# nekopanda/Amatsukaze

Hardware: AMD Instinct MI355X
Metric: frames/sec 1440x1080i logo+CM+KFM pass (higher is better)
Workload: dtype f32; 1 GPU; configs[1]: 10000x 1440x1080i 8-bit in HBM: AMTAnalyzeLogo, LogoFrame scan x3, CM/KFM metrics, CalcFade, AMTEraseLogo; analysis_mode=linear, library_default_mode=exact, calc_fade=device, erase=into a resident writable copy (MakeWritable's frame), frames_per_gpu=10000, logo=256x128@(1120,64), parallelism=single GPU

## Files before the change

### amatsukaze_amd/build.py

```python
from __future__ import annotations

import os
import subprocess
import sys

HERE = os.path.dirname(os.path.abspath(__file__))
CSRC = os.path.join(HERE, "csrc")
OUT = os.path.join(HERE, "libamt_gpu.so")

SOURCES = [
    "amt_gpu.hip",
    "amt_gpu_erase_scan.hip",
    "amt_gpu_stats.hip",
    "amt_gpu_ingest.hip",
    "amt_gpu_upload.hip",
    "eval_engine.hip",
    "eval_fused_kernels.hip",
    "eval_linear_kernels.hip",
    "eval_pair_kernels.hip",
    "eval_pair1_kernels.hip",
    "erase_scan_kernels.hip",
    "erase_surface_kernels.hip",
    "stats_kernels.hip",
    "stats_msb_kernels.hip",
    "ingest_kernels.hip",
    "amt_gpu_logofind.hip",
    "logofind_kernels.hip",
    "logofind_msb_kernels.hip",
    "surface_kernels.hip",
    "amt_gpu_audio.hip",
    "audio_kernels.hip",
    "amt_gpu_render.hip",
    "render_kernels.hip",
    "render_surface_kernels.hip",
    "render_adaptive_kernels.hip",
    "render_adaptive_surface_kernels.hip",
    "amt_gpu_tnr.hip",
    "temporal_nr_kernels.hip",
    "temporal_nr_surface_kernels.hip",
    "amt_gpu_resize.hip",
    "resize_kernels.hip",
    "resize_surface_kernels.hip",
    "resize_plan.cpp",
    "amt_gpu_deband.hip",
    "deband_kernels.hip",
    "deband_surface_kernels.hip",
    "deband_plan.cpp",
    "amt_gpu_edgelevel.hip",
    "edgelevel_kernels.hip",
    "logo_model.cpp",
    "logo_fit.cpp",
    "decisions.cpp",
    "stats_decisions.cpp",
    "amts_file.cpp",
    "logo_find.cpp",
]

FLAGS = ["--offload-arch=gfx950", "-O3", "-std=c++17", "-fPIC", "-ffp-contract=off", "-fno-fast-math",
         "-fgpu-rdc" if False else "-fno-gpu-rdc", "-Wall", "-Wno-unused-function", "-Wno-unused-result"]


EXTRA_FLAGS = {"eval_fused_kernels.hip": ["-mllvm", "-amdgpu-sched-strategy=max-ilp"],
               "eval_linear_kernels.hip": ["-fno-slp-vectorize"]}


def hipcc() -> str:
    for c in (os.environ.get("HIPCC"), "/opt/rocm/bin/hipcc", "hipcc"):
        if c and (os.path.isabs(c) and os.path.exists(c) or not os.path.isabs(c)):
            return c
    raise RuntimeError("hipcc not found")


def needs_build(srcs) -> bool:
# ... 64 lines not shown
```

### amatsukaze_amd/csrc/engine.hpp

```cpp
#pragma once

#include <hip/hip_runtime.h>

#include <cstdint>
#include <mutex>
#include <utility>
#include <stdexcept>
#include <string>
#include <vector>

#include "eval_plan.h"
#include "eval_tiles.hpp"
#include "kernels.hpp"
#include "logo_model.hpp"

#define AMT_HIP(expr)                                                                              \
    do {                                                                                           \
        hipError_t e_ = (expr);                                                                    \
        if (e_ != hipSuccess)                                                                      \
            throw std::runtime_error(std::string(#expr) + ": " + hipGetErrorString(e_));          \
    } while (0)

#ifdef AMT_TRACE_CALLS
#include <chrono>
// ... 97 lines not shown
};

struct EvalLogoSpec {
    LogoPlanes planes;
    MaskTables tables;
    int imgx = 0, imgy = 0;
    int row0 = 0, row_step = 1, deint = 1;
    int out_off = 0;
};

class EvalEngine {
public:
    EvalEngine(AmtGpuContext* ctx, std::vector<EvalLogoSpec> specs, std::vector<float> fades, bool take_abs, int out_frame_stride,
               const char* prof_name = "logo_eval_fused_kernel");
    void run(const FrameBatch& luma, int bits, int nframes, float* dout, const int* dframe_map = nullptr);
    void run_linear(const FrameBatch& luma, int bits, int nframes, float* dout, const int* dframe_map = nullptr, uint8_t* dforce = nullptr);
    void set_linear_queue(int entries) { lin_queue_ = entries; }
    float linear_error_bound(int logo, int bits) const;
    void run_listed(const FrameBatch& luma, int bits, int max_frames, const int* dlist, const int* dcount, float* dout, int G = 1,
                    int fade_chunk = -1);
    int exact_group_frames(int nframes) const;
    int num_fades() const { return (int)fades_.size(); }
    int num_logos() const { return (int)specs_.size(); }
    const EvalLogoSpec& spec(int i) const { return specs_[i]; }
    double mask_pixel_evals_per_frame() const;

private:
    AmtGpuContext* ctx_;
    std::vector<EvalLogoSpec> specs_;
    std::vector<float> fades_;
    bool take_abs_;
    int out_frame_stride_;
    std::string prof_name_;
    int plane_cap_ = 0;
    int group_frames_ = 0;
    std::vector<EvalBand> bands_;
    std::vector<DevBuf<float>> d_a_, d_b_;
    std::vector<DevBuf<float2>> d_scales_, d_kslot_;
    std::vector<DevBuf<uint2>> d_slot2_;
    DevBuf<EvalLogoDev> d_logos_;
    DevBuf<EvalBand> d_bands_;
    DevBuf<float> d_fades_;
    bool pair_eligible();
    bool pair_addressable(int pitch_bytes) const;
    bool tiles_usable(int pitch_bytes) const;
    int pair_state_ = -1;
    void ensure_tiles();
    bool tiles_ready_ = false;
    bool tile_slots_ok_ = true;
    static bool stage4_eligible(const EvalLogoSpec& S);
    bool tiles_stage4_ = false;
    std::vector<DevBuf<float2>> d_tkp_, d_tsc_, d_tpq_;
    bool tiles_units_ = false;
    std::vector<DevBuf<uint32_t>> d_tinfo_, d_tpos_, d_tunits_;
    std::vector<DevBuf<char>> d_tlin_;
    int lin_queue_ = 256;
    std::vector<DevBuf<TileDesc>> d_tiles_;
    std::vector<DevBuf<TileBandDesc>> d_tbands_;
    std::vector<DevBuf<int>> d_tlist_;
    DevBuf<TileLogoDev> d_tls_;
    void ensure_linear();
    bool linear_ready_ = false;
    float vmax_unit_ = 1.0f;
    std::vector<double> lin_err_corr_, lin_err_sum_;
    std::vector<double> lin_err_formula_;
    bool lin_formula_ok_ = true;
};

}
```

### amatsukaze_amd/csrc/eval_engine.hip

```cpp
#include "build_knobs.h"
#include "engine.hpp"
#include "exact_math.h"

#include <algorithm>
#include <cmath>
#include <cstring>

int AmtGpuContext::prof_id(const char* name)
{
    for (size_t i = 0; i < prof_names.size(); ++i) if (prof_names[i] == name) return (int)i;
    prof_names.push_back(name);
    prof_ms.push_back(0.0);
    prof_calls.push_back(0);
    return (int)prof_names.size() - 1;
}
hipEvent_t AmtGpuContext::prof_event()
{
    if (!prof_pool.empty()) { hipEvent_t e = prof_pool.back(); prof_pool.pop_back(); return e; }
    hipEvent_t e;
    AMT_HIP(hipEventCreate(&e));
    return e;
}
int AmtGpuContext::prof_begin(const char* name)
{
// ... 110 lines not shown
            for (int sidx = B.s0; sidx < B.s0 + B.nslots; ++sidx) {
                const int m0 = slot_m0(sidx);
                const int n = (int)(slots[sidx] >> 28);
                const int x = (int)(T.pos[m0] & 0xFFFF), y = (int)(T.pos[m0] >> 16);
                slot2[sidx] = uint2{slots[sidx], (uint32_t)((y - 2 - B.y0) * B.lp + (x - 2 - B.x0))};
                const float* k0 = &T.kernels[(size_t)m0 * 25];
                const float* k1 = n > 1 ? &T.kernels[(size_t)(m0 + 1) * 25] : nullptr;
                for (int c = 0; c < 5; ++c)
                    for (int r = 0; r < 5; ++r) {
                        const float a0 = c < 4 ? k0[r * 5 + c + 1] : k0[r * 5];
                        const float a1 = k1 ? (c < 4 ? k1[r * 5 + c] : k1[r * 5 + 4]) : 0.0f;
                        kslot[(size_t)(c * 5 + r) * spad + sidx] = float2{a0, a1};
                    }
            }
        }
        d_a_[i].upload(S.planes.A(0), (size_t)w * h, ctx_->stream);
        d_b_[i].upload(S.planes.B(0), (size_t)w * h, ctx_->stream);
        d_scales_[i].upload(scales, ctx_->stream);
        d_kslot_[i].upload(kslot, ctx_->stream);
        d_slot2_[i].upload(slot2, ctx_->stream);

        EvalLogoDev& D = hl[i];
        D.a = d_a_[i].get(); D.b = d_b_[i].get(); D.scales = d_scales_[i].get();
        D.kslot = d_kslot_[i].get(); D.slot2 = d_slot2_[i].get(); D.nslots_pad = spad;
        D.band0 = band0; D.nbands = (int)bands_.size() - band0;
        D.w = w; D.h = h; D.count = T.count; D.count_pad = cpad;
        D.imgx = S.imgx; D.imgy = S.imgy; D.row0 = S.row0; D.row_step = S.row_step; D.deint = S.deint;
        D.blackScore = T.blackScore;
        D.out_off = S.out_off;
        D.lp = lp;
    }
    d_logos_.upload(hl, ctx_->stream);
    d_bands_.upload(bands_, ctx_->stream);
    d_fades_.upload(fades_, ctx_->stream);
}

double EvalEngine::mask_pixel_evals_per_frame() const
{
    double s = 0;
    for (const auto& sp : specs_) s += (double)sp.tables.count * fades_.size();
    return s;
}

void EvalEngine::run(const FrameBatch& luma, int bits, int nframes, float* dout, const int* dframe_map)
{
    if (nframes <= 0 || specs_.empty()) return;
    ctx_->bind();
    const int nl = (int)specs_.size();
    int G = exact_group_frames(nframes);
    const int nf_all = (int)fades_.size();
    if (pair_eligible() && pair_addressable(luma.pitchY * luma.es)) {
        const size_t dot = prof_name_.find('.');
        const std::string suffix = dot == std::string::npos ? std::string() : prof_name_.substr(dot);
        const int Gp = group_frames_ > 0 ? group_frames_ : (int)std::max(1LL, std::min((long long)kTileMaxFrames, (long long)nframes * nl / 2048));
        const int sp = ctx_->prof_begin(((tiles_stage4_ ? "logo_eval_pair_kernel" : "logo_eval_pair_ldexp_kernel") + suffix).c_str());
        AMT_HIP((tiles_units_ ? launch_logo_eval_pair1 : launch_logo_eval_pair)(ctx_->stream, bits, d_logos_.get(), d_tls_.get(), nl, luma, dframe_map, nframes, Gp, dout, out_frame_stride_,
                                      take_abs_ ? 1 : 0, tiles_stage4_ ? 0 : 1));
        ctx_->prof_end(sp);
        return;
    }
    for (int f0 = 0; f0 < nf_all; f0 += kEvalMaxFades) {
        const int nf = std::min(kEvalMaxFades, nf_all - f0);
        G = std::max(1, std::min(G, kEvalThreads / nf));
        const int sp = ctx_->prof_begin(prof_name_.c_str());
        AMT_HIP(launch_logo_eval_fused(ctx_->stream, bits, d_logos_.get(), nl, d_bands_.get(), d_fades_.get(), nf, f0, luma, dframe_map, nframes, G,
                                       dout, out_frame_stride_, take_abs_ ? 1 : 0, plane_cap_));
        ctx_->prof_end(sp);
    }
}

int EvalEngine::exact_group_frames(int nframes) const
{
    const int nl = (int)specs_.size();
    return group_frames_ > 0 ? group_frames_ : (int)std::max(1LL, std::min(8LL, (long long)nframes * nl / 2048));
}

bool EvalEngine::pair_eligible()
{
    if (pair_state_ >= 0) return pair_state_ == 1;
    pair_state_ = 0;
    if (fades_.size() != 2 || fades_[0] != 0.0f || fades_[1] != 1.0f || specs_.empty()) return false;
    for (const EvalLogoSpec& S : specs_) {
        const int w = S.planes.w, h = S.planes.h;
        if (w < 6 || (w & 1) || h < 5 || S.tables.count <= 0 || S.tables.count >= (1 << 20)) return false;
        if (!S.deint) return false;
        const float* a = S.planes.A(0);
        const float* b = S.planes.B(0);
        for (int p = 0; p < w * h; ++p)
            if (!(std::fabs(a[p]) + std::fabs(b[p]) < 8192.0f)) return false;
    }
    ensure_tiles();
    if (!tile_slots_ok_) return false;
    pair_state_ = 1;
    return true;
}

bool EvalEngine::pair_addressable(int pitch_bytes) const
{
    for (const EvalLogoSpec& S : specs_) {
        const long long last_row = (long long)S.imgy + S.row0 + (long long)S.planes.h * S.row_step + 1;
        const long long last = last_row * pitch_bytes + (long long)(S.imgx + S.planes.w) * 2;
        if (last >= (1LL << 31) || pitch_bytes <= 0) return false;
        if ((long long)S.imgy + S.row0 < 0 || !tile_mul24_operands_ok(pitch_bytes, S.row_step, last_row, S.planes.w, S.planes.h)) return false;
    }
    return true;
}

bool EvalEngine::stage4_eligible(const EvalLogoSpec& S)
{
    if (!S.deint) return false;
    const float* a = S.planes.A(0);
    const float* b = S.planes.B(0);
    const size_t npx = (size_t)S.planes.w * S.planes.h;
    for (size_t p = 0; p < npx; ++p)
        if (!stage4_coef_ok(a[p], b[p])) return false;
    const MaskTables& T = S.tables;
    for (int m = 0; m < T.count; ++m) {
        const float* k = &T.kernels[(size_t)m * 25];
        float ksum = 0.0f;
        for (int t = 0; t < 25; ++t) {
            ksum += k[t];
            if (!stage4_tap_ok(k[t])) return false;
        }
        if (!stage4_tap_ok(ksum)) return false;
    }
    return true;
}

void EvalEngine::ensure_tiles()
{
    if (tiles_ready_) return;
    ctx_->bind();
    const int nl = (int)specs_.size();
    std::vector<TileLogoDev> hl(nl);
    tiles_stage4_ = fades_.size() == 2;
    for (const EvalLogoSpec& S : specs_) tiles_stage4_ = tiles_stage4_ && stage4_eligible(S);
    std::vector<TilePlan> plans(nl);
    for (int i = 0; i < nl; ++i)
        plans[i] = build_tile_plan(specs_[i].tables.pos, specs_[i].tables.count, specs_[i].planes.w, specs_[i].planes.h,
                                   fades_.size() == 2 ? kTileCutBest : kTileCutCoarse);
    tiles_units_ = false;
    if (fades_.size() == 2) {
        std::vector<TilePlan> single(nl);
        for (int i = 0; i < nl; ++i)
            single[i] = build_tile_plan(specs_[i].tables.pos, specs_[i].tables.count, specs_[i].planes.w, specs_[i].planes.h, kTileCutUnits);
        tiles_units_ = tile_plans_single_pass(plans, single);
        if (tiles_units_) plans.swap(single);
    }
    d_tunits_.resize(nl);
    d_tkp_.resize(nl); d_tsc_.resize(nl); d_tpq_.resize(nl); d_tinfo_.resize(nl); d_tpos_.resize(nl); d_tlin_.resize(nl); d_tiles_.resize(nl); d_tbands_.resize(nl); d_tlist_.resize(nl);
    for (int i = 0; i < nl; ++i) {
        const EvalLogoSpec& S = specs_[i];
        const MaskTables& T = S.tables;
        const TilePlan& P = plans[i];
        if (!tile_slots_ok(P.nslots())) { tile_slots_ok_ = false; continue; }
        const size_t ns = (size_t)P.nslots();
        const float kscale = tiles_stage4_ ? 0.25f : 1.0f;
        std::vector<float2> kp(13 * ns, float2{0.0f, 0.0f}), sc((size_t)kNumBins * ns, float2{0.0f, 0.0f}), pq(ns, float2{0.0f, 0.0f});
        std::vector<uint32_t> spos(ns, 0u);
        for (size_t s = 0; s < ns; ++s) {
            const int m = P.slot_pixel[s];
            if (m < 0) continue;
            fit_response(&T.resp[(size_t)m * 32], pq[s].x, pq[s].y);
            spos[s] = T.pos[m];
            const float* k = &T.kernels[(size_t)m * 25];
            float ksum = 0.0f;
            if (fades_.size() == 2) {
                for (int t = 0; t < 25; ++t) ksum += k[t];
            } else {
                double ks = 0.0;
                for (int t = 0; t < 25; ++t) ks += (double)k[t];
                ksum = (float)ks;
            }
            for (int j = 0; j < 13; ++j) kp[(size_t)j * ns + s] = float2{kscale * k[2 * j], kscale * (2 * j + 1 < 25 ? k[2 * j + 1] : ksum)};
            for (int c = 0; c < kNumBins; ++c)
                sc[(size_t)c * ns + s] = float2{T.scales[((size_t)m * 32 + c) * 2], T.scales[((size_t)m * 32 + c) * 2 + 1]};
        }
        d_tkp_[i].upload(kp, ctx_->stream);
        d_tsc_[i].upload(sc, ctx_->stream);
        d_tpq_[i].upload(pq, ctx_->stream);
        d_tpos_[i].upload(spos, ctx_->stream);
        const size_t npx = (size_t)S.planes.w * S.planes.h;
        const size_t o_pq = kp.size() * sizeof(float2), o_si = o_pq + pq.size() * sizeof(float2), o_a = o_si + P.sinfo.size() * sizeof(uint32_t),
                     o_b = o_a + npx * sizeof(float), total = o_b + npx * sizeof(float);
        if (total >= ((size_t)1 << 31)) throw std::runtime_error("logo too large");
        std::vector<char> blob(total);
        std::memcpy(blob.data(), kp.data(), o_pq);
        std::memcpy(blob.data() + o_pq, pq.data(), o_si - o_pq);
        std::memcpy(blob.data() + o_si, P.sinfo.data(), o_a - o_si);
        std::memcpy(blob.data() + o_a, S.planes.A(0), npx * sizeof(float));
        std::memcpy(blob.data() + o_b, S.planes.B(0), npx * sizeof(float));
        d_tlin_[i].upload(blob, ctx_->stream);
        d_tinfo_[i].upload(P.sinfo, ctx_->stream);
        d_tiles_[i].upload(P.tiles, ctx_->stream);
        d_tbands_[i].upload(P.bands, ctx_->stream);
        std::vector<int> tlist;
        for (size_t t = 0; t < P.tiles.size(); ++t) if (P.tiles[t].npix > 0) tlist.push_back((int)t);
        d_tlist_[i].upload(tlist, ctx_->stream);
        hl[i] = TileLogoDev{d_tkp_[i].get(), d_tsc_[i].get(), d_tpq_[i].get(), d_tinfo_[i].get(), d_tpos_[i].get(), d_tiles_[i].get(), d_tbands_[i].get(), d_tlist_[i].get(),
                            (int)P.bands.size(), (int)ns, (int)tlist.size(), T.floorResp};
// ... 138 lines not shown
```

### amatsukaze_amd/csrc/eval_pair_body.h

```cpp
#pragma once
#include "build_knobs.h"
#include <hip/hip_runtime.h>
#include <cstdint>
#include <algorithm>
#include <type_traits>

#include "engine.hpp"
#include "eval_tiles.hpp"
#include "exact_math.h"
#include "eval_tile_stage.h"
#include "eval_ordered_sum.h"

namespace amt {

using namespace lin;
using namespace tile;

constexpr int kPairThreads = (kTileWaves + 1) * 64;
constexpr int kPairRowPitch = kTileBandPix + kEvalScorePad;

__device__ __forceinline__ f2 window_corr_exact(const f2 (&Kp)[13], const f2 (&W)[25], f2 M)
{
    f2 p[5];
#pragma unroll
    for (int i = 0; i < 5; ++i) {
        f2 t[5];
#pragma unroll
        for (int r = 0; r < 5; ++r) {
            const int e = r * 5 + i;
            const f2 kk = (e & 1) ? bc_hi(Kp[e >> 1]) : bc_lo(Kp[e >> 1]);
            t[r] = kk * (W[e] - M);
        }
        p[i] = ((t[0] + t[1]) + (t[2] + t[3])) + t[4];
    }
    return ((p[0] + p[4]) + p[2]) + (p[1] + p[3]);
}

template <bool STAGE4> __device__ __forceinline__ unsigned score_bin_bounded(float mean)
{
    return STAGE4 ? (unsigned)((int)__builtin_amdgcn_fmed3f(mean, 0.0f, 1020.0f) >> 5) : (unsigned)((int)__builtin_amdgcn_fmed3f(mean, 0.0f, 255.0f) >> 3);
}

struct PairLaunch {
    const EvalLogoDev* logos;
    const TileLogoDev* tls;
    const void* Y;
    const int* frame_map;
    long long frame_stride;
    int pitch;
    float maxv;
    int nframes, G, ngroups, nlogos;
    float* out;
    int out_frame_stride, take_abs;
};

#ifdef AMT_PAIR_OCC
#define AMT_PAIR_OCC_ATTR __attribute__((amdgpu_waves_per_eu(AMT_PAIR_OCC, AMT_PAIR_OCC)))
#else
#define AMT_PAIR_OCC_ATTR
#endif
template <typename pix_t, bool STAGE4, bool ONE_UNIT = false>
__device__ __forceinline__ void logo_eval_pair_body(const PairLaunch& A)
{
    extern __shared__ float lds[];
    f2* const planes = reinterpret_cast<f2*>(lds);
    float* const rows = lds + kTileWaves * kTileCap * 2;

    const int G = A.G;
    const WgMap wm = wg_map_shared_rows((int)blockIdx.x, A.nlogos, A.ngroups);
    if (wm.grp >= A.ngroups) return;
    const int logo = wm.logo, grp = wm.grp;
    const int F0 = grp * G;
    const int gcount = min(G, A.nframes - F0);
    const int tid = threadIdx.x, lane = tid & 63;
    const int wave = __builtin_amdgcn_readfirstlane(tid >> 6);
    const EvalLogoDev* const Lp = A.logos + logo;
    const TileLogoDev* const Xp = A.tls + logo;
    const int nbands = Xp->nbands;

    if (wave == kTileWaves) {
        __builtin_amdgcn_s_setprio(3);
        float acc = 0.0f;
        typedef const __attribute__((address_space(4))) TileBandDesc* const_band_ptr;
        const const_band_ptr bd = (const_band_ptr)Xp->bands;
        for (int b = 0; b < nbands; ++b) {
            asm volatile("s_waitcnt lgkmcnt(0)\n\ts_barrier" ::: "memory");
            const int npix = bd[b].npix;
            if (lane < 2 * gcount) acc = ordered_row_sum(rows + ((b & 1) * 2 * G + lane) * kPairRowPitch, npix, acc);
        }
        if (lane < 2 * gcount) {
            float r = acc / Lp->blackScore;
            if (A.take_abs) r = fabsf(r);
            A.out[(long long)(F0 + (lane >> 1)) * A.out_frame_stride + Lp->out_off + (lane & 1)] = r;
        }
        return;
    }

    typedef const __attribute__((address_space(4))) TileLogoDev* tlogo_ptr;
    const gptr_t gSc = (gptr_t)Xp->sc, gK = (gptr_t)((tlogo_ptr)Xp)->kp, gInfo = (gptr_t)((tlogo_ptr)Xp)->sinfo;
    const unsigned nslots8 = (unsigned)Xp->nslots * 8u;
    const const_tile_ptr tiles = (const_tile_ptr)(Xp->tiles + wave);
    f2* const myplane = planes + wave * kTileCap;
    const unsigned plane_base = lds_address(myplane);
    typename std::conditional<ONE_UNIT, TileStager1<pix_t, STAGE4>, TileStager<pix_t, STAGE4>>::type st;
    st.init(Lp, A.pitch, A.maxv, myplane);
    TilePixel px;

    TileDesc T;
    fetch_tile(T, tiles);
    gptr_t gUnits = nullptr;
    unsigned unext = 0;
    if constexpr (ONE_UNIT) {
        gUnits = (gptr_t)((tlogo_ptr)Xp)->units;
        st.setup_units(T, gld<unsigned>(gUnits, ((unsigned)wave * 64u + (unsigned)lane) * 4u));
    } else {
        st.setup_units(T, lane);
    }
    st.request(frame_rsrc<pix_t>(A.Y, A.frame_map, A.frame_stride, F0));
    asm volatile("" ::: "memory");
    if constexpr (ONE_UNIT) unext = gld<unsigned>(gUnits, ((unsigned)((nbands > 1 ? kTileWaves : 0) + wave) * 64u + (unsigned)lane) * 4u);
    px.load(gK, gInfo, nslots8, (unsigned)wave * 64u + (unsigned)lane, T, plane_base);
    if constexpr (ONE_UNIT) asm volatile("" : "+v"(unext));
    st.coefs_landed();

    f2 pR = {0.0f, 0.0f}, psc0 = pR, psc1 = pR;
    int prow = 0;
    bool pact = false;
    auto flush_terms = [&]() {
        if (pact) {
            float* const pdst = rows + prow * kPairRowPitch + px.ridx;
            pdst[0] = score_term(pR.x, psc0.x, psc0.y);
            pdst[kPairRowPitch] = score_term(pR.y, psc1.x, psc1.y);
        }
    };

    int b = 0, g = 0;
    const int niter = nbands * gcount;
    for (int it = 0; it < niter; ++it) {
        const bool band_end = g + 1 == gcount;
        st.convert();
        if (band_end && b + 1 < nbands) {
            fetch_tile(T, tiles + (b + 1) * kTileWaves);
            if constexpr (ONE_UNIT) st.setup_units(T, unext);
            else st.setup_units(T, lane);
        }
        st.request(frame_rsrc<pix_t>(A.Y, A.frame_map, A.frame_stride, F0 + (band_end ? 0 : g + 1)));
#pragma unroll
        for (int j = 0; j < 13; ++j) asm volatile("" : "+v"(px.Kp[j]));
        f2 W[25];
        unsigned wrow[5];
        px.rows(wrow);
        const f2 M = window_load_means(wrow, W);
        const f2 R = window_corr_exact(px.Kp, W, M);
        flush_terms();
        psc0 = gld<f2>(gSc, __umul24(score_bin_bounded<STAGE4>(M.x), nslots8) + px.slot8);
        psc1 = gld<f2>(gSc, __umul24(score_bin_bounded<STAGE4>(M.y), nslots8) + px.slot8);
        pR = R; pact = px.act;
        prow = (b & 1) * 2 * G + g * 2;
        if (band_end) {
            flush_terms();
            pact = false;
            ++b; g = 0;
            if (b < nbands) {
                st.coefs_landed();
                if constexpr (ONE_UNIT) unext = gld<unsigned>(gUnits, ((unsigned)((b + 1 < nbands ? b + 1 : b) * kTileWaves + wave) * 64u + (unsigned)lane) * 4u);
                px.load(gK, gInfo, nslots8, (unsigned)(b * kTileWaves + wave) * 64u + (unsigned)lane, T, plane_base);
                if constexpr (ONE_UNIT) asm volatile("" : "+v"(unext));
            }
            asm volatile("s_waitcnt lgkmcnt(0)\n\ts_barrier" ::: "memory");
        } else {
            ++g;
        }
    }
}

inline hipError_t pair_launch_args(PairLaunch& A, size_t* lds, unsigned* grid, int bits, const EvalLogoDev* dlogos, const TileLogoDev* dtls, int nlogos,
                                   const FrameBatch& luma, const int* dframe_map, int nframes, int G, float* dout, int out_frame_stride, int take_abs)
{
    *grid = 0; *lds = 0;
    if (nframes <= 0 || nlogos <= 0) return hipSuccess;
    if (luma.shift || luma.es != (bits <= 8 ? 1 : 2)) return hipErrorInvalidValue;
    A.logos = dlogos; A.tls = dtls; A.Y = luma.Y; A.frame_map = dframe_map; A.frame_stride = luma.strideY / luma.es; A.pitch = luma.pitchY;
    A.maxv = (float)((1 << bits) - 1);
    A.nframes = nframes; A.G = G; A.ngroups = (nframes + G - 1) / G; A.nlogos = nlogos;
    A.out = dout; A.out_frame_stride = out_frame_stride; A.take_abs = take_abs;
    *lds = ((size_t)kTileWaves * kTileCap * 2 + (size_t)2 * 2 * G * kPairRowPitch) * sizeof(float);
    if (G < 1 || 2 * G > 64 || *lds > 160 * 1024) return hipErrorInvalidValue;
    *grid = (unsigned)wg_grid_shared_rows(A.ngroups, nlogos);
    return hipSuccess;
}

}
```

### amatsukaze_amd/csrc/eval_tiles.hpp

```cpp
#pragma once

#include <algorithm>
#include <cstdint>
#include <stdexcept>
#include <vector>

namespace amt {

#ifndef AMT_TILE_WAVES
#define AMT_TILE_WAVES 11
#endif
constexpr int kTileWaves = AMT_TILE_WAVES;
#ifndef AMT_TILE_G
#define AMT_TILE_G 8
#endif
constexpr int kTileMaxFrames = AMT_TILE_G;
constexpr int kTileLanes = 64;
constexpr int kTileBandPix = kTileWaves * kTileLanes;
constexpr int kTileCap = 512;
constexpr int kTileUnits = kTileCap / 4 / kTileLanes;

struct TileDesc {
    int x0, y0;
    int nrows, ncol4;
// ... 12 lines not shown
#endif
AMT_TILE_HD unsigned mul24(unsigned a, unsigned b)
{
#if defined(__HIP_DEVICE_COMPILE__)
    return __umul24(a, b);
#else
    return a * b;
#endif
}
constexpr long long kMul24Limit = 1LL << 24;
constexpr long long kTileSlotLimit = 1LL << 20;
inline bool tile_mul24_operands_ok(long long pitch_bytes, long long row_step, long long last_row, long long w, long long h)
{
    return pitch_bytes > 0 && pitch_bytes < kMul24Limit && row_step >= 1 && row_step < kMul24Limit &&
           last_row >= 0 && last_row < kMul24Limit && w > 0 && w <= 65536 && h > 0 && h <= 65536;
}
inline bool tile_slots_ok(long long nslots) { return nslots >= 0 && nslots < kTileSlotLimit; }

struct TileUnit { int y, xs, lds; };
AMT_TILE_HD TileUnit tile_unit(const TileDesc& T, int u, int w)
{
    const int last = T.nrows * T.ncol4 - 1;
    u = u < last ? u : (last < 0 ? 0 : last);
    const int row = (int)(mul24((unsigned)u, (unsigned)T.rcp) >> 16);
    const int c4 = u - (int)mul24((unsigned)row, (unsigned)T.ncol4);
    const int x = T.x0 + 4 * c4;
    const int xs = x < w - 4 ? x : w - 4;
    return TileUnit{T.y0 + row, xs, (int)mul24((unsigned)row, (unsigned)T.tp) + (xs - T.x0)};
}
AMT_TILE_HD unsigned tile_unit_word(int row, int c4) { return ((unsigned)row << 8) | (unsigned)c4; }
AMT_TILE_HD TileUnit tile_unit_listed(const TileDesc& T, unsigned word, int w)
{
    const int row = (int)(word >> 8), c4 = (int)(word & 0xFFu);
    const int x = T.x0 + 4 * c4;
    const int xs = x < w - 4 ? x : w - 4;
    return TileUnit{T.y0 + row, xs, (int)mul24((unsigned)row, (unsigned)T.tp) + (xs - T.x0)};
}

constexpr int kXcds = 8;
struct WgMap { int logo, grp; };
AMT_TILE_HD WgMap wg_map_shared_rows(int bid, int nlogos, int ngroups)
{
    (void)ngroups;
    const int x = bid & (kXcds - 1), r = bid >> 3;
    const int blk = r / nlogos;
    return WgMap{r - blk * nlogos, blk * kXcds + x};
}
inline long long wg_grid_shared_rows(long long ngroups, int nlogos) { return (ngroups + kXcds - 1) / kXcds * kXcds * nlogos; }

inline uint32_t tile_slot_info(int woff, int ridx, bool valid) { return (uint32_t)woff | ((uint32_t)ridx << 12) | (valid ? 0x80000000u : 0u); }

struct TilePlan {
    std::vector<TileBandDesc> bands;
    std::vector<TileDesc> tiles;
    std::vector<uint32_t> sinfo;
    std::vector<int> slot_pixel;
    long long model_cost = 0;
    int nslots() const { return (int)sinfo.size(); }
    std::vector<uint32_t> units;
    std::vector<int> nunits;
    bool single_pass = false;
};
enum TileCut { kTileCutCoarse, kTileCutFine, kTileCutBest, kTileCutUnits };

namespace tiles_detail {

struct Px { int x, y, m; };

inline int split_lanes(const std::vector<Px>& g, int x0, int y0, int tp, std::vector<uint8_t>* half)
{
    const int n = (int)g.size();
    int k[32] = {0};
    std::vector<int> bank(n);
    for (int i = 0; i < n; ++i) { bank[i] = ((g[i].y - 2 - y0) * tp + (g[i].x - 2 - x0)) & 31; ++k[bank[i]]; }
    for (int total = 2;; ++total)
        for (int ca = (total + 1) / 2; ca < total; ++ca) {
            const int cb = total - ca;
            int lo = 0, hi = 0;
            bool ok = true;
            for (int b = 0; b < 32; ++b) { ok = ok && k[b] <= total; lo += std::max(0, k[b] - cb); hi += std::min(k[b], ca); }
            const int smin = std::max(lo, n - 32), smax = std::min(hi, 32);
            if (!ok || smin > smax) continue;
            if (half) {
                int a[32], sum = 0;
                for (int b = 0; b < 32; ++b) { a[b] = std::max(0, k[b] - cb); sum += a[b]; }
                const int want = std::min(std::max((n + 1) / 2, smin), smax);
                for (bool moved = true; sum < want && moved;) {
                    moved = false;
                    for (int b = 0; b < 32 && sum < want; ++b)
                        if (a[b] < std::min(k[b], ca)) { ++a[b]; ++sum; moved = true; }
                }
                half->assign(n, 1);
                for (int i = 0; i < n; ++i)
                    if (a[bank[i]] > 0) { (*half)[i] = 0; --a[bank[i]]; }
            }
            return total;
        }
}

struct Geometry { int x0, y0, nrows, ncol4; };
inline Geometry bbox(const std::vector<Px>& g, size_t a, size_t b)
{
    int xmin = 1 << 30, xmax = -1, ymin = 1 << 30, ymax = -1;
    for (size_t i = a; i < b; ++i) {
        xmin = std::min(xmin, g[i].x); xmax = std::max(xmax, g[i].x);
        ymin = std::min(ymin, g[i].y); ymax = std::max(ymax, g[i].y);
    }
    Geometry G;
    G.x0 = (xmin - 2) & ~1;
    G.y0 = ymin - 2;
    G.nrows = ymax + 2 - G.y0 + 1;
    G.ncol4 = (xmax + 2 - G.x0 + 1 + 3) / 4;
    return G;
}
inline bool fits(const Geometry& G) { return G.nrows * G.ncol4 * 4 <= kTileCap && G.nrows * G.ncol4 <= kTileLanes * kTileUnits; }
inline void add_needed_units(std::vector<uint32_t>& keys, int x0, const Px& p)
{
    for (int y = p.y - 2; y <= p.y + 2; ++y)
        for (int c4 = (p.x - 2 - x0) / 4; c4 <= (p.x + 2 - x0) / 4; ++c4) {
            const uint32_t key = ((uint32_t)y << 8) | (uint32_t)c4;
            if (std::find(keys.begin(), keys.end(), key) == keys.end()) keys.push_back(key);
        }
}

}

namespace tiles_detail {

inline std::vector<std::vector<Px>> deal_band(const std::vector<uint32_t>& pos, int m, int n, bool units = false)
{
    std::vector<Px> px(n);
    for (int i = 0; i < n; ++i) px[i] = Px{(int)(pos[m + i] & 0xFFFFu), (int)(pos[m + i] >> 16), m + i};
    std::stable_sort(px.begin(), px.end(), [](const Px& a, const Px& b) { return a.x < b.x; });
    std::vector<std::vector<Px>> groups;
    for (size_t a = 0; a < px.size();) {
        size_t b = a + 1;
        std::vector<uint32_t> keys;
        const int x0 = (px[a].x - 2) & ~1;
        if (units) add_needed_units(keys, x0, px[a]);
        while (b < px.size() && b - a < (size_t)kTileLanes && fits(bbox(px, a, b + 1))) {
            if (units) {
                add_needed_units(keys, x0, px[b]);
                if (keys.size() > (size_t)kTileLanes) break;
            }
            ++b;
        }
        groups.emplace_back(px.begin() + a, px.begin() + b);
        a = b;
    }
    return groups;
}
inline std::vector<int> cut_bands(const std::vector<uint32_t>& pos, int count, bool fine, bool units = false)
{
    std::vector<int> cuts;
    for (int m = 0; m < count;) {
        int n = std::min(kTileBandPix, count - m);
        while ((int)deal_band(pos, m, n, units).size() > kTileWaves)
            n = fine ? std::max(1, n - 4) : std::max(1, n - std::max(1, n / 8));
        cuts.push_back(n);
        m += n;
    }
    if (fine && cuts.size() >= 2 && cuts.back() < kTileLanes) {
        const int n = cuts[cuts.size() - 2] + cuts.back();
        if (n <= kTileBandPix && (int)deal_band(pos, count - n, n, units).size() <= kTileWaves) { cuts.pop_back(); cuts.back() = n; }
    }
    return cuts;
}

}

inline TilePlan build_tile_plan(const std::vector<uint32_t>& pos, int count, int w, int h, TileCut cut = kTileCutCoarse)
{
    using namespace tiles_detail;
    (void)h;
    if (w < 5) throw std::runtime_error("logo too narrow for the tile kernel");
    if (cut == kTileCutBest) {
        TilePlan coarse = build_tile_plan(pos, count, w, h, kTileCutCoarse), fine = build_tile_plan(pos, count, w, h, kTileCutFine);
        return fine.model_cost < coarse.model_cost ? fine : coarse;
    }
    TilePlan P;
    const bool units = cut == kTileCutUnits;
    P.single_pass = units;
    int m = 0;
    for (const int n : cut_bands(pos, count, cut == kTileCutFine || units, units)) {
        std::vector<std::vector<Px>> groups = deal_band(pos, m, n, units);
        {
            std::vector<size_t> order(groups.size());
            for (size_t i = 0; i < order.size(); ++i) order[i] = i;
            auto cost = [&](size_t i) { const Geometry G = bbox(groups[i], 0, groups[i].size()); return 131 + 31 * (!units && G.nrows * G.ncol4 > kTileLanes ? 2 : 1); };
            std::stable_sort(order.begin(), order.end(), [&](size_t a, size_t b) { return cost(a) > cost(b); });
            int load[4] = {0, 0, 0, 0}, used[4] = {0, 0, 0, 0}, cap[4] = {0, 0, 0, 0};
            for (int w = 0; w < kTileWaves; ++w) ++cap[w % 4];
            std::vector<std::vector<Px>> placed(kTileWaves);
            for (size_t i : order) {
                int best = -1;
                for (int k = 0; k < 4; ++k)
                    if (used[k] < cap[k] && (best < 0 || load[k] < load[best])) best = k;
                placed[best + 4 * used[best]] = groups[i];
                load[best] += cost(i); ++used[best];
            }
            P.model_cost += *std::max_element(load, load + 4);
            groups.swap(placed);
        }
        const int band = (int)P.bands.size();
        P.bands.push_back(TileBandDesc{m, n});
        P.tiles.resize((size_t)(band + 1) * kTileWaves, TileDesc{0, 0, 0, 1, 4, 0, 65536, 0});
        P.sinfo.resize((size_t)(band + 1) * kTileBandPix, tile_slot_info(0, 0, false));
        P.slot_pixel.resize((size_t)(band + 1) * kTileBandPix, -1);
        if (units) {
            P.units.resize((size_t)(band + 1) * kTileBandPix, tile_unit_word(0, 0));
            P.nunits.resize((size_t)(band + 1) * kTileWaves, 0);
        }
        for (size_t gi = 0; gi < groups.size(); ++gi) {
            const std::vector<Px>& g = groups[gi];
            if (g.empty()) continue;
            const Geometry G = bbox(g, 0, g.size());
            int best_tp = G.ncol4 * 4, best_cyc = 1 << 30;
            for (int tp = G.ncol4 * 4; tp * G.nrows <= kTileCap && tp < G.ncol4 * 4 + 32; tp += 2) {
                const int c = split_lanes(g, G.x0, G.y0, tp, nullptr);
                if (c < best_cyc) { best_cyc = c; best_tp = tp; }
            }
            std::vector<uint8_t> half;
            split_lanes(g, G.x0, G.y0, best_tp, &half);
            TileDesc& T = P.tiles[(size_t)band * kTileWaves + gi];
            T.x0 = G.x0; T.y0 = G.y0; T.nrows = G.nrows; T.ncol4 = G.ncol4; T.tp = best_tp; T.npix = (int)g.size();
            T.rcp = (65536 + G.ncol4 - 1) / G.ncol4;
            for (int u = 0; u < kTileLanes * kTileUnits; ++u)
                if (((u * T.rcp) >> 16) != u / G.ncol4) throw std::runtime_error("tile plan: unit row magic");
            int next[2] = {0, kTileLanes / 2}, filler[2] = {-1, -1};
            for (size_t i = 0; i < g.size(); ++i) {
                const int l = next[half[i]]++;
                const size_t slot = ((size_t)band * kTileWaves + gi) * kTileLanes + l;
                const int woff = (g[i].y - 2 - G.y0) * best_tp + (g[i].x - 2 - G.x0);
                if (l >= kTileLanes / 2 * (half[i] + 1)) throw std::runtime_error("tile plan: more than 32 pixels in half a wave");
                if (woff < 0 || woff + 4 * best_tp + 4 > G.nrows * best_tp - 1 || G.nrows * best_tp > kTileCap) throw std::runtime_error("tile plan: window outside its tile");
                P.sinfo[slot] = tile_slot_info(woff, g[i].m - m, true);
                P.slot_pixel[slot] = g[i].m;
                if (filler[half[i]] < 0) filler[half[i]] = woff;
            }
            for (int hf = 0; hf < 2; ++hf) {
                const int woff = filler[hf] >= 0 ? filler[hf] : filler[1 - hf];
                for (int l = next[hf]; l < kTileLanes / 2 * (hf + 1); ++l)
                    P.sinfo[((size_t)band * kTileWaves + gi) * kTileLanes + l] = tile_slot_info(woff, 0, false);
            }
            if (units) {
                std::vector<uint32_t> keys;
                for (const Px& p : g) add_needed_units(keys, G.x0, p);
                if (keys.empty() || keys.size() > (size_t)kTileLanes) throw std::runtime_error("tile plan: needed units");
                for (uint32_t& k : keys) k = tile_unit_word((int)(k >> 8) - G.y0, (int)(k & 0xFFu));
                std::sort(keys.begin(), keys.end());
                const size_t tile = (size_t)band * kTileWaves + gi;
                P.nunits[tile] = (int)keys.size();
                for (int l = 0; l < kTileLanes; ++l) P.units[tile * kTileLanes + l] = keys[std::min((size_t)l, keys.size() - 1)];
            }
        }
        m += n;
    }
    return P;
}

inline bool tile_plans_single_pass(const std::vector<TilePlan>& best, const std::vector<TilePlan>& units)
{
    if (best.empty() || best.size() != units.size()) return false;
    for (size_t i = 0; i < best.size(); ++i)
        if (!units[i].single_pass || units[i].model_cost > best[i].model_cost || !tile_slots_ok(units[i].nslots())) return false;
    return true;
}

}
```

### amatsukaze_amd/csrc/kernels.hpp

```cpp
#pragma once

#include <hip/hip_runtime.h>
#include <cstdint>

#include "eval_plan.h"
#include "frame_batch.h"
#include "lane_rule.h"
#include "resize_region.h"

namespace amt {

struct TileDesc; struct TileBandDesc;

struct PlanesOut { void *Y, *U, *V; };
struct ScanRect { int imgx, imgy, cx, cy, w, h, wUV, hUV; };
inline ScanRect scan_rect(int imgx, int imgy, int w, int h) { return ScanRect{imgx, imgy, imgx >> 1, imgy >> 1, w, h, w >> 1, h >> 1}; }

template <typename F> inline void with_sample_type(int bits, F&& f) { bits <= 8 ? f(uint8_t()) : f(uint16_t()); }

struct EraseGeom {
    int w, h, wUV, hUV;
    int imgx, imgy, cx, cy;
    int uvparity;
};
// ... 176 lines not shown
struct EdgeLevelGrid { int spans, units, luma_blocks; dim3 grid; };
inline bool edgelevel_grid(const EdgeLevelArgs& a, int nframes, EdgeLevelGrid& g)
{
    if ((a.es != 1 && a.es != 2) || a.W <= 0 || a.H <= 0 || (a.W & 1) || (a.H & 1) || nframes <= 0) return false;
    if (a.strength < 0 || a.strength > 255 || a.thresh < 0 || a.repair < 0 || a.repair > 4) return false;
    if (!a.srcY || !a.srcU || !a.srcV || !a.dstY || !a.dstU || !a.dstV) return false;
    if (a.src_pitchY < a.W * a.es || a.dst_pitchY < a.W * a.es || a.src_pitchUV < a.W / 2 * a.es || a.dst_pitchUV < a.W / 2 * a.es) return false;
    const long long spans = ((long long)a.W * a.es + kEdgeSpanBytes - 1) / kEdgeSpanBytes, strips = (a.H + kEdgeStripRows - 1) / kEdgeStripRows;
    const long long units = spans * strips, luma_blocks = (units + 3) / 4, chroma_blocks = (a.H + 3) / 4;
    if (units > 0x7FFFFFF0LL || luma_blocks + chroma_blocks > 0x7FFFFFFFLL) return false;
    g = EdgeLevelGrid{(int)spans, (int)units, (int)luma_blocks, dim3((unsigned)(luma_blocks + chroma_blocks), (unsigned)(nframes < 65535 ? nframes : 65535))};
    return true;
}
hipError_t launch_edgelevel(hipStream_t st, const EdgeLevelArgs& a, int nframes);

hipError_t launch_frame_stats(hipStream_t st, int bits, const FrameBatch& b, int W, int H, const void* dprevY, int nframes, unsigned long long* dout);
long long logofind_launch_cap(int bits);
hipError_t launch_logofind(hipStream_t st, int bits, const FrameBatch& b, int W, int H, int nframes, int num_cus, unsigned long long* dS1,
                           unsigned long long* dSM);

struct AudioTimeline { long long num_samples, step_num, fps_num; int channels; };
constexpr int kAudioLevelWords = 4;
hipError_t launch_audio_levels(hipStream_t st, const int16_t* dpcm, long long pcm_first, const AudioTimeline& t, long long first_frame,
                               int nframes, unsigned long long* dout);

struct TileLogoDev {
    const float2* kp;
    const float2* sc;
    const float2* pq;
    const uint32_t* sinfo;
    const uint32_t* pos;
    const TileDesc* tiles;
    const TileBandDesc* bands;
    const int* tlist;
    int nbands, nslots, ntlist;
    float floorResp;
    const char* lin;
    unsigned lin_pq, lin_sinfo, lin_a, lin_b;
    const uint32_t* units;
};
hipError_t launch_logo_eval_fused(hipStream_t st, int bits, const EvalLogoDev* dlogos, int nlogos, const EvalBand* dbands,
                                  const float* dfades, int nfades, int fade0, const FrameBatch& luma, const int* dframe_map, int nframes, int G,
                                  float* dout, int out_frame_stride, int take_abs, int plane_cap, const int* dnframes = nullptr, int scatter = 0,
                                  int fade_chunk = 0);
hipError_t launch_logo_eval_linear(hipStream_t st, int bits, const EvalLogoDev* dlogos, const TileLogoDev* dtls, int nlogos,
                                   const float* dfades, int nfades, int fade0, const FrameBatch& luma, const int* dframe_map, int nframes, int G,
                                   float* dout, int out_frame_stride, int take_abs, float bin_eps, int qlog2, int qcap, uint8_t* dforce);
hipError_t launch_logo_eval_pair(hipStream_t st, int bits, const EvalLogoDev* dlogos, const TileLogoDev* dtls, int nlogos,
                                 const FrameBatch& luma, const int* dframe_map, int nframes, int G, float* dout, int out_frame_stride, int take_abs,
                                 int ldexp_form);
hipError_t launch_logo_eval_pair1(hipStream_t st, int bits, const EvalLogoDev* dlogos, const TileLogoDev* dtls, int nlogos,
                                  const FrameBatch& luma, const int* dframe_map, int nframes, int G, float* dout, int out_frame_stride, int take_abs,
                                  int ldexp_form);
struct MonitorState {
    unsigned max_abs_bits;
    int tripped;
    unsigned long long frames_checked;
    unsigned batches_tripped;
    unsigned pad_;
};
struct SentinelArgs {
    int nsent = 0;
    float* side = nullptr;
    uint8_t* side_forced = nullptr;
    int* gate = nullptr;
};
hipError_t launch_analysis_mark(hipStream_t st, const float* drec, int stride, int nframes, int ngroups, int nfades, const float* eps3,
                                int* dlist, int* dcount, const uint8_t* dforce = nullptr, const SentinelArgs& sent = SentinelArgs());
hipError_t launch_analysis_sentinel_check(hipStream_t st, const float* drec, int stride, int nframes, const SentinelArgs& sent, float tol,
                                          MonitorState* dstate, int* host_flag, int epoch);
hipError_t launch_analysis_iota(hipStream_t st, int* dlist, int n);
hipError_t launch_rect_range_flag(hipStream_t st, const FrameBatch& luma, int imgx, int imgy, int w, int h, int bits, int nframes, uint8_t* dflag);

}
```

Baseline: 1.324 million frames/sec.

## Add seven-wave duo variant of single-pass pair eval kernel with smaller frame groups

Adds a new pair-eval kernel shape that uses 7 compute waves per workgroup and at most 6 frames per group, pinned to 4 waves per EU, with tile plans rebuilt for the narrower band width. A host-side selector chooses it when LDS fits and the total work cost spread over four SIMDs does not exceed the existing plan's critical-path cost. The aim is higher occupancy and better SIMD balance in logo evaluation. In exchange there are more bands, more workgroups and less frame reuse per workgroup.

```diff
diff --git a/amatsukaze_amd/build.py b/amatsukaze_amd/build.py
--- a/amatsukaze_amd/build.py
+++ b/amatsukaze_amd/build.py
@@ -19,6 +19,7 @@
     "eval_linear_kernels.hip",
     "eval_pair_kernels.hip",
     "eval_pair1_kernels.hip",
+    "eval_pair1_duo_kernels.hip",
     "erase_scan_kernels.hip",
     "erase_surface_kernels.hip",
     "stats_kernels.hip",
diff --git a/amatsukaze_amd/csrc/engine.hpp b/amatsukaze_amd/csrc/engine.hpp
--- a/amatsukaze_amd/csrc/engine.hpp
+++ b/amatsukaze_amd/csrc/engine.hpp
@@ -173,6 +173,7 @@
     bool tiles_stage4_ = false;
     std::vector<DevBuf<float2>> d_tkp_, d_tsc_, d_tpq_;
     bool tiles_units_ = false;
+    PairShape pair_shape_{kTileWaves, kTileMaxFrames, false};
     std::vector<DevBuf<uint32_t>> d_tinfo_, d_tpos_, d_tunits_;
     std::vector<DevBuf<char>> d_tlin_;
     int lin_queue_ = 256;
diff --git a/amatsukaze_amd/csrc/eval_engine.hip b/amatsukaze_amd/csrc/eval_engine.hip
--- a/amatsukaze_amd/csrc/eval_engine.hip
+++ b/amatsukaze_amd/csrc/eval_engine.hip
@@ -186,9 +186,11 @@
     if (pair_eligible() && pair_addressable(luma.pitchY * luma.es)) {
         const size_t dot = prof_name_.find('.');
         const std::string suffix = dot == std::string::npos ? std::string() : prof_name_.substr(dot);
-        const int Gp = group_frames_ > 0 ? group_frames_ : (int)std::max(1LL, std::min((long long)kTileMaxFrames, (long long)nframes * nl / 2048));
+        const bool duo = pair_shape_.duo;
+        const int Gw = group_frames_ > 0 ? group_frames_ : (int)std::max(1LL, std::min((long long)kTileMaxFrames, (long long)nframes * nl / 2048));
+        const int Gp = duo ? std::min(Gw, pair_shape_.frames) : Gw;
         const int sp = ctx_->prof_begin(((tiles_stage4_ ? "logo_eval_pair_kernel" : "logo_eval_pair_ldexp_kernel") + suffix).c_str());
-        AMT_HIP((tiles_units_ ? launch_logo_eval_pair1 : launch_logo_eval_pair)(ctx_->stream, bits, d_logos_.get(), d_tls_.get(), nl, luma, dframe_map, nframes, Gp, dout, out_frame_stride_,
+        AMT_HIP((duo ? launch_logo_eval_pair1_duo : tiles_units_ ? launch_logo_eval_pair1 : launch_logo_eval_pair)(ctx_->stream, bits, d_logos_.get(), d_tls_.get(), nl, luma, dframe_map, nframes, Gp, dout, out_frame_stride_,
                                       take_abs_ ? 1 : 0, tiles_stage4_ ? 0 : 1));
         ctx_->prof_end(sp);
         return;
@@ -279,7 +281,15 @@
         for (int i = 0; i < nl; ++i)
             single[i] = build_tile_plan(specs_[i].tables.pos, specs_[i].tables.count, specs_[i].planes.w, specs_[i].planes.h, kTileCutUnits);
         tiles_units_ = tile_plans_single_pass(plans, single);
-        if (tiles_units_) plans.swap(single);
+        std::vector<TilePlan> duo(nl);
+        for (int i = 0; i < nl; ++i)
+            duo[i] = build_tile_plan(specs_[i].tables.pos, specs_[i].tables.count, specs_[i].planes.w, specs_[i].planes.h, kTileCutUnits, kPairDuoWaves);
+        int dev = 0, lds_limit = 0;
+        AMT_HIP(hipGetDevice(&dev));
+        AMT_HIP(hipDeviceGetAttribute(&lds_limit, hipDeviceAttributeMaxSharedMemoryPerBlock, dev));
+        pair_shape_ = tile_pair_shape(plans, single, duo, (size_t)std::max(0, lds_limit), kEvalScorePad);
+        if (pair_shape_.duo) { tiles_units_ = true; plans.swap(duo); }
+        else if (tiles_units_) plans.swap(single);
     }
     d_tunits_.resize(nl);
     d_tkp_.resize(nl); d_tsc_.resize(nl); d_tpq_.resize(nl); d_tinfo_.resize(nl); d_tpos_.resize(nl); d_tlin_.resize(nl); d_tiles_.resize(nl); d_tbands_.resize(nl); d_tlist_.resize(nl);
diff --git a/amatsukaze_amd/csrc/eval_pair1_duo_kernels.hip b/amatsukaze_amd/csrc/eval_pair1_duo_kernels.hip
--- /dev/null
+++ b/amatsukaze_amd/csrc/eval_pair1_duo_kernels.hip
@@ -0,0 +1,37 @@
+#include "build_knobs.h"
+#include "eval_pair_body.h"
+
+namespace amt {
+
+constexpr int kPairDuoThreads = pair_threads(kPairDuoWaves);
+#define AMT_PAIR_DUO_ATTR __launch_bounds__(kPairDuoThreads) __attribute__((amdgpu_waves_per_eu(4, 4)))
+
+template <typename pix_t>
+__global__ AMT_PAIR_DUO_ATTR
+void logo_eval_pair1_duo_kernel(const PairLaunch A) { logo_eval_pair_body<pix_t, true, true, kPairDuoWaves>(A); }
+template <typename pix_t>
+__global__ AMT_PAIR_DUO_ATTR
+void logo_eval_pair1_duo_ldexp_kernel(const PairLaunch A) { logo_eval_pair_body<pix_t, false, true, kPairDuoWaves>(A); }
+
+hipError_t launch_logo_eval_pair1_duo(hipStream_t st, int bits, const EvalLogoDev* dlogos, const TileLogoDev* dtls, int nlogos,
+                                      const FrameBatch& luma, const int* dframe_map,
+                                      int nframes, int G, float* dout, int out_frame_stride, int take_abs, int ldexp_form)
+{
+    PairLaunch A;
+    size_t lds;
+    unsigned nwg;
+    if (G > kPairDuoFrames) return hipErrorInvalidValue;
+    const hipError_t e = pair_launch_args(A, &lds, &nwg, bits, dlogos, dtls, nlogos, luma, dframe_map, nframes, G, dout, out_frame_stride, take_abs, kPairDuoWaves);
+    if (e != hipSuccess || nwg == 0) return e;
+    dim3 grid(nwg);
+    if (ldexp_form) {
+        if (bits <= 8) hipLaunchKernelGGL(logo_eval_pair1_duo_ldexp_kernel<uint8_t>, grid, dim3(kPairDuoThreads), lds, st, A);
+        else hipLaunchKernelGGL(logo_eval_pair1_duo_ldexp_kernel<uint16_t>, grid, dim3(kPairDuoThreads), lds, st, A);
+    } else {
+        if (bits <= 8) hipLaunchKernelGGL(logo_eval_pair1_duo_kernel<uint8_t>, grid, dim3(kPairDuoThreads), lds, st, A);
+        else hipLaunchKernelGGL(logo_eval_pair1_duo_kernel<uint16_t>, grid, dim3(kPairDuoThreads), lds, st, A);
+    }
+    return hipGetLastError();
+}
+
+}
diff --git a/amatsukaze_amd/csrc/eval_pair_body.h b/amatsukaze_amd/csrc/eval_pair_body.h
--- a/amatsukaze_amd/csrc/eval_pair_body.h
+++ b/amatsukaze_amd/csrc/eval_pair_body.h
@@ -16,8 +16,9 @@
 using namespace lin;
 using namespace tile;
 
-constexpr int kPairThreads = (kTileWaves + 1) * 64;
-constexpr int kPairRowPitch = kTileBandPix + kEvalScorePad;
+constexpr int pair_threads(int nw) { return (nw + 1) * 64; }
+constexpr int pair_row_pitch(int nw) { return nw * kTileLanes + kEvalScorePad; }
+constexpr int kPairThreads = pair_threads(kTileWaves);
 
 __device__ __forceinline__ f2 window_corr_exact(const f2 (&Kp)[13], const f2 (&W)[25], f2 M)
 {
@@ -59,12 +60,13 @@
 #else
 #define AMT_PAIR_OCC_ATTR
 #endif
-template <typename pix_t, bool STAGE4, bool ONE_UNIT = false>
+template <typename pix_t, bool STAGE4, bool ONE_UNIT = false, int NW = kTileWaves>
 __device__ __forceinline__ void logo_eval_pair_body(const PairLaunch& A)
 {
+    constexpr int kPairRowPitch = pair_row_pitch(NW);
     extern __shared__ float lds[];
     f2* const planes = reinterpret_cast<f2*>(lds);
-    float* const rows = lds + kTileWaves * kTileCap * 2;
+    float* const rows = lds + NW * kTileCap * 2;
 
     const int G = A.G;
     const WgMap wm = wg_map_shared_rows((int)blockIdx.x, A.nlogos, A.ngroups);
@@ -78,7 +80,7 @@
     const TileLogoDev* const Xp = A.tls + logo;
     const int nbands = Xp->nbands;
 
-    if (wave == kTileWaves) {
+    if (wave == NW) {
         __builtin_amdgcn_s_setprio(3);
         float acc = 0.0f;
         typedef const __attribute__((address_space(4))) TileBandDesc* const_band_ptr;
@@ -118,7 +120,7 @@
     }
     st.request(frame_rsrc<pix_t>(A.Y, A.frame_map, A.frame_stride, F0));
     asm volatile("" ::: "memory");
-    if constexpr (ONE_UNIT) unext = gld<unsigned>(gUnits, ((unsigned)((nbands > 1 ? kTileWaves : 0) + wave) * 64u + (unsigned)lane) * 4u);
+    if constexpr (ONE_UNIT) unext = gld<unsigned>(gUnits, ((unsigned)((nbands > 1 ? NW : 0) + wave) * 64u + (unsigned)lane) * 4u);
     px.load(gK, gInfo, nslots8, (unsigned)wave * 64u + (unsigned)lane, T, plane_base);
     if constexpr (ONE_UNIT) asm volatile("" : "+v"(unext));
     st.coefs_landed();
@@ -140,7 +142,7 @@
         const bool band_end = g + 1 == gcount;
         st.convert();
         if (band_end && b + 1 < nbands) {
-            fetch_tile(T, tiles + (b + 1) * kTileWaves);
+            fetch_tile(T, tiles + (b + 1) * NW);
             if constexpr (ONE_UNIT) st.setup_units(T, unext);
             else st.setup_units(T, lane);
         }
@@ -163,8 +165,8 @@
             ++b; g = 0;
             if (b < nbands) {
                 st.coefs_landed();
-                if constexpr (ONE_UNIT) unext = gld<unsigned>(gUnits, ((unsigned)((b + 1 < nbands ? b + 1 : b) * kTileWaves + wave) * 64u + (unsigned)lane) * 4u);
-                px.load(gK, gInfo, nslots8, (unsigned)(b * kTileWaves + wave) * 64u + (unsigned)lane, T, plane_base);
+                if constexpr (ONE_UNIT) unext = gld<unsigned>(gUnits, ((unsigned)((b + 1 < nbands ? b + 1 : b) * NW + wave) * 64u + (unsigned)lane) * 4u);
+                px.load(gK, gInfo, nslots8, (unsigned)(b * NW + wave) * 64u + (unsigned)lane, T, plane_base);
                 if constexpr (ONE_UNIT) asm volatile("" : "+v"(unext));
             }
             asm volatile("s_waitcnt lgkmcnt(0)\n\ts_barrier" ::: "memory");
@@ -175,7 +177,8 @@
 }
 
 inline hipError_t pair_launch_args(PairLaunch& A, size_t* lds, unsigned* grid, int bits, const EvalLogoDev* dlogos, const TileLogoDev* dtls, int nlogos,
-                                   const FrameBatch& luma, const int* dframe_map, int nframes, int G, float* dout, int out_frame_stride, int take_abs)
+                                   const FrameBatch& luma, const int* dframe_map, int nframes, int G, float* dout, int out_frame_stride, int take_abs,
+                                   int nw = kTileWaves)
 {
     *grid = 0; *lds = 0;
     if (nframes <= 0 || nlogos <= 0) return hipSuccess;
@@ -184,7 +187,7 @@
     A.maxv = (float)((1 << bits) - 1);
     A.nframes = nframes; A.G = G; A.ngroups = (nframes + G - 1) / G; A.nlogos = nlogos;
     A.out = dout; A.out_frame_stride = out_frame_stride; A.take_abs = take_abs;
-    *lds = ((size_t)kTileWaves * kTileCap * 2 + (size_t)2 * 2 * G * kPairRowPitch) * sizeof(float);
+    *lds = tile_pair_lds_bytes(nw, G, kEvalScorePad);
     if (G < 1 || 2 * G > 64 || *lds > 160 * 1024) return hipErrorInvalidValue;
     *grid = (unsigned)wg_grid_shared_rows(A.ngroups, nlogos);
     return hipSuccess;
diff --git a/amatsukaze_amd/csrc/eval_tiles.hpp b/amatsukaze_amd/csrc/eval_tiles.hpp
--- a/amatsukaze_amd/csrc/eval_tiles.hpp
+++ b/amatsukaze_amd/csrc/eval_tiles.hpp
@@ -88,10 +88,12 @@
 
 struct TilePlan {
     std::vector<TileBandDesc> bands;
+    int waves = kTileWaves;
     std::vector<TileDesc> tiles;
     std::vector<uint32_t> sinfo;
     std::vector<int> slot_pixel;
     long long model_cost = 0;
+    long long work_cost = 0;
     int nslots() const { return (int)sinfo.size(); }
     std::vector<uint32_t> units;
     std::vector<int> nunits;
@@ -186,39 +188,43 @@
     }
     return groups;
 }
-inline std::vector<int> cut_bands(const std::vector<uint32_t>& pos, int count, bool fine, bool units = false)
+inline std::vector<int> cut_bands(const std::vector<uint32_t>& pos, int count, bool fine, bool units = false, int nw = kTileWaves)
 {
     std::vector<int> cuts;
+    const int band_pix = nw * kTileLanes;
     for (int m = 0; m < count;) {
-        int n = std::min(kTileBandPix, count - m);
-        while ((int)deal_band(pos, m, n, units).size() > kTileWaves)
+        int n = std::min(band_pix, count - m);
+        while ((int)deal_band(pos, m, n, units).size() > nw)
             n = fine ? std::max(1, n - 4) : std::max(1, n - std::max(1, n / 8));
         cuts.push_back(n);
         m += n;
     }
     if (fine && cuts.size() >= 2 && cuts.back() < kTileLanes) {
         const int n = cuts[cuts.size() - 2] + cuts.back();
-        if (n <= kTileBandPix && (int)deal_band(pos, count - n, n, units).size() <= kTileWaves) { cuts.pop_back(); cuts.back() = n; }
+        if (n <= band_pix && (int)deal_band(pos, count - n, n, units).size() <= nw) { cuts.pop_back(); cuts.back() = n; }
     }
     return cuts;
 }
 
 }
 
-inline TilePlan build_tile_plan(const std::vector<uint32_t>& pos, int count, int w, int h, TileCut cut = kTileCutCoarse)
+inline TilePlan build_tile_plan(const std::vector<uint32_t>& pos, int count, int w, int h, TileCut cut = kTileCutCoarse, int nw = kTileWaves)
 {
     using namespace tiles_detail;
     (void)h;
     if (w < 5) throw std::runtime_error("logo too narrow for the tile kernel");
     if (cut == kTileCutBest) {
-        TilePlan coarse = build_tile_plan(pos, count, w, h, kTileCutCoarse), fine = build_tile_plan(pos, count, w, h, kTileCutFine);
+        TilePlan coarse = build_tile_plan(pos, count, w, h, kTileCutCoarse, nw), fine = build_tile_plan(pos, count, w, h, kTileCutFine, nw);
         return fine.model_cost < coarse.model_cost ? fine : coarse;
     }
     TilePlan P;
     const bool units = cut == kTileCutUnits;
     P.single_pass = units;
+    P.waves = nw;
+    if (nw < 1 || nw > 15) throw std::runtime_error("tile plan: waves per band");
+    const int band_pix = nw * kTileLanes;
     int m = 0;
-    for (const int n : cut_bands(pos, count, cut == kTileCutFine || units, units)) {
+    for (const int n : cut_bands(pos, count, cut == kTileCutFine || units, units, nw)) {
         std::vector<std::vector<Px>> groups = deal_band(pos, m, n, units);
         {
             std::vector<size_t> order(groups.size());
@@ -226,26 +232,27 @@
             auto cost = [&](size_t i) { const Geometry G = bbox(groups[i], 0, groups[i].size()); return 131 + 31 * (!units && G.nrows * G.ncol4 > kTileLanes ? 2 : 1); };
             std::stable_sort(order.begin(), order.end(), [&](size_t a, size_t b) { return cost(a) > cost(b); });
             int load[4] = {0, 0, 0, 0}, used[4] = {0, 0, 0, 0}, cap[4] = {0, 0, 0, 0};
-            for (int w = 0; w < kTileWaves; ++w) ++cap[w % 4];
-            std::vector<std::vector<Px>> placed(kTileWaves);
+            for (int w = 0; w < nw; ++w) ++cap[w % 4];
+            std::vector<std::vector<Px>> placed(nw);
             for (size_t i : order) {
                 int best = -1;
                 for (int k = 0; k < 4; ++k)
                     if (used[k] < cap[k] && (best < 0 || load[k] < load[best])) best = k;
                 placed[best + 4 * used[best]] = groups[i];
                 load[best] += cost(i); ++used[best];
+                P.work_cost += cost(i);
             }
             P.model_cost += *std::max_element(load, load + 4);
             groups.swap(placed);
         }
         const int band = (int)P.bands.size();
         P.bands.push_back(TileBandDesc{m, n});
-        P.tiles.resize((size_t)(band + 1) * kTileWaves, TileDesc{0, 0, 0, 1, 4, 0, 65536, 0});
-        P.sinfo.resize((size_t)(band + 1) * kTileBandPix, tile_slot_info(0, 0, false));
-        P.slot_pixel.resize((size_t)(band + 1) * kTileBandPix, -1);
+        P.tiles.resize((size_t)(band + 1) * nw, TileDesc{0, 0, 0, 1, 4, 0, 65536, 0});
+        P.sinfo.resize((size_t)(band + 1) * band_pix, tile_slot_info(0, 0, false));
+        P.slot_pixel.resize((size_t)(band + 1) * band_pix, -1);
         if (units) {
-            P.units.resize((size_t)(band + 1) * kTileBandPix, tile_unit_word(0, 0));
-            P.nunits.resize((size_t)(band + 1) * kTileWaves, 0);
+            P.units.resize((size_t)(band + 1) * band_pix, tile_unit_word(0, 0));
+            P.nunits.resize((size_t)(band + 1) * nw, 0);
         }
         for (size_t gi = 0; gi < groups.size(); ++gi) {
             const std::vector<Px>& g = groups[gi];
@@ -258,7 +265,7 @@
             }
             std::vector<uint8_t> half;
             split_lanes(g, G.x0, G.y0, best_tp, &half);
-            TileDesc& T = P.tiles[(size_t)band * kTileWaves + gi];
+            TileDesc& T = P.tiles[(size_t)band * nw + gi];
             T.x0 = G.x0; T.y0 = G.y0; T.nrows = G.nrows; T.ncol4 = G.ncol4; T.tp = best_tp; T.npix = (int)g.size();
             T.rcp = (65536 + G.ncol4 - 1) / G.ncol4;
             for (int u = 0; u < kTileLanes * kTileUnits; ++u)
@@ -266,7 +273,7 @@
             int next[2] = {0, kTileLanes / 2}, filler[2] = {-1, -1};
             for (size_t i = 0; i < g.size(); ++i) {
                 const int l = next[half[i]]++;
-                const size_t slot = ((size_t)band * kTileWaves + gi) * kTileLanes + l;
+                const size_t slot = ((size_t)band * nw + gi) * kTileLanes + l;
                 const int woff = (g[i].y - 2 - G.y0) * best_tp + (g[i].x - 2 - G.x0);
                 if (l >= kTileLanes / 2 * (half[i] + 1)) throw std::runtime_error("tile plan: more than 32 pixels in half a wave");
                 if (woff < 0 || woff + 4 * best_tp + 4 > G.nrows * best_tp - 1 || G.nrows * best_tp > kTileCap) throw std::runtime_error("tile plan: window outside its tile");
@@ -277,7 +284,7 @@
             for (int hf = 0; hf < 2; ++hf) {
                 const int woff = filler[hf] >= 0 ? filler[hf] : filler[1 - hf];
                 for (int l = next[hf]; l < kTileLanes / 2 * (hf + 1); ++l)
-                    P.sinfo[((size_t)band * kTileWaves + gi) * kTileLanes + l] = tile_slot_info(woff, 0, false);
+                    P.sinfo[((size_t)band * nw + gi) * kTileLanes + l] = tile_slot_info(woff, 0, false);
             }
             if (units) {
                 std::vector<uint32_t> keys;
@@ -285,7 +292,7 @@
                 if (keys.empty() || keys.size() > (size_t)kTileLanes) throw std::runtime_error("tile plan: needed units");
                 for (uint32_t& k : keys) k = tile_unit_word((int)(k >> 8) - G.y0, (int)(k & 0xFFu));
                 std::sort(keys.begin(), keys.end());
-                const size_t tile = (size_t)band * kTileWaves + gi;
+                const size_t tile = (size_t)band * nw + gi;
                 P.nunits[tile] = (int)keys.size();
                 for (int l = 0; l < kTileLanes; ++l) P.units[tile * kTileLanes + l] = keys[std::min((size_t)l, keys.size() - 1)];
             }
@@ -295,12 +302,34 @@
     return P;
 }
 
-inline bool tile_plans_single_pass(const std::vector<TilePlan>& best, const std::vector<TilePlan>& units)
+inline bool tile_plans_single_pass(const std::vector<TilePlan>& best, const std::vector<TilePlan>& units, int nw = kTileWaves)
 {
     if (best.empty() || best.size() != units.size()) return false;
     for (size_t i = 0; i < best.size(); ++i)
-        if (!units[i].single_pass || units[i].model_cost > best[i].model_cost || !tile_slots_ok(units[i].nslots())) return false;
+        if (!units[i].single_pass || units[i].waves != nw || best[i].waves != nw || units[i].model_cost > best[i].model_cost || !tile_slots_ok(units[i].nslots())) return false;
     return true;
 }
 
-}
+inline size_t tile_pair_lds_bytes(int nw, int G, int row_pad)
+{
+    return ((size_t)nw * kTileCap * 2 + (size_t)2 * 2 * G * (nw * kTileLanes + row_pad)) * sizeof(float);
+}
+
+constexpr int kPairDuoWaves = 7;
+constexpr int kPairDuoFrames = 6;
+struct PairShape { int waves, frames; bool duo; };
+
+inline PairShape tile_pair_shape(const std::vector<TilePlan>& best, const std::vector<TilePlan>& units, const std::vector<TilePlan>& duo,
+                                 size_t lds_per_workgroup, int row_pad)
+{
+    const PairShape keep{kTileWaves, kTileMaxFrames, false};
+    if (best.empty() || best.size() != units.size() || best.size() != duo.size()) return keep;
+    if (tile_pair_lds_bytes(kPairDuoWaves, kPairDuoFrames, row_pad) > lds_per_workgroup) return keep;
+    for (size_t i = 0; i < best.size(); ++i) {
+        const long long existing = units[i].single_pass ? std::min(best[i].model_cost, units[i].model_cost) : best[i].model_cost;
+        if (!duo[i].single_pass || duo[i].waves != kPairDuoWaves || !tile_slots_ok(duo[i].nslots()) || (duo[i].work_cost + 3) / 4 > existing) return keep;
+    }
+    return PairShape{kPairDuoWaves, kPairDuoFrames, true};
+}
+
+}
diff --git a/amatsukaze_amd/csrc/kernels.hpp b/amatsukaze_amd/csrc/kernels.hpp
--- a/amatsukaze_amd/csrc/kernels.hpp
+++ b/amatsukaze_amd/csrc/kernels.hpp
@@ -252,6 +252,9 @@
 hipError_t launch_logo_eval_pair1(hipStream_t st, int bits, const EvalLogoDev* dlogos, const TileLogoDev* dtls, int nlogos,
                                   const FrameBatch& luma, const int* dframe_map, int nframes, int G, float* dout, int out_frame_stride, int take_abs,
                                   int ldexp_form);
+hipError_t launch_logo_eval_pair1_duo(hipStream_t st, int bits, const EvalLogoDev* dlogos, const TileLogoDev* dtls, int nlogos,
+                                      const FrameBatch& luma, const int* dframe_map, int nframes, int G, float* dout, int out_frame_stride, int take_abs,
+                                      int ldexp_form);
 struct MonitorState {
     unsigned max_abs_bits;
     int tripped;
```

New measurement: 1.362 million frames/sec, median of 6. 2.8% higher.
